# vmoens/mujoco-torch

Hardware: AMD Instinct MI355X
Metric: env-steps/sec (higher is better)
Workload: dtype f64

## Files before the change

mujoco-torch_amd/csrc/mjh_kernels.h:

```cpp
#pragma once
#include <cstring>
#include "mjh_device.h"

template <typename REAL>
struct LdsView {
  REAL* base;
  const LdsOff* off;
#define X(n, c, p) __device__ __forceinline__ REAL* n() const { return base + off->n; }
  MJH_LDS_ARRAYS(X, _)
#undef X
};

#ifndef MJH_NO_NT
#define MJH_NT_STORE(v, p) __builtin_nontemporal_store((v), (p))
#else
#define MJH_NT_STORE(v, p) (*(p) = (v))
#endif
template <typename MM>
inline int lds_carve(const MM& m, int phase_bit, LdsOff& o, int* kv_defer_ok = nullptr) {
  int off = 0;
#define X(n, c, p) o.n = off; if ((p) & phase_bit) off += (((c) + 1) & ~1);
  MJH_LDS_ARRAYS(X, m)
#undef X
  if (phase_bit == PH_CON) {
// ... 1543 lines not shown
          b[0] = 0; b[1] = 0; b[2] = 0;
          if ((REAL)-0.5 < n[1] && n[1] < (REAL)0.5) b[1] = 1; else b[2] = 1;
        }
        REAL c[3];
        cross3(n, b, c);
#pragma unroll
        for (int i = 0; i < 3; i++) { frame[i] = n[i]; frame[3 + i] = b[i]; frame[6 + i] = c[i]; }
        const REAL seg[3] = {axis[0] * s2[1], axis[1] * s2[1], axis[2] * s2[1]};
#pragma unroll
        for (int q = 0; q < 2; q++) {
          REAL sp[3];
#pragma unroll
          for (int i = 0; i < 3; i++) sp[i] = p2[i] + (q == 0 ? seg[i] : -seg[i]);
          plane_sphere_(n, p1, sp, s2[0], dist[q], pos[q]);
        }
      } else if (fn == MJH_FN_SPHERE_SPHERE) {
        REAL n[3];
        sphere_sphere_(p1, s1[0], p2, s2[0], dist[0], pos[0], n);
        make_frame(n, frame);
      } else if (fn == MJH_FN_SPHERE_CAPSULE) {
        const REAL axis[3] = {m2[2], m2[5], m2[8]};
        REAL a[3], b[3], pt[3], n[3];
#pragma unroll
        for (int i = 0; i < 3; i++) { REAL sg = axis[i] * s2[1]; a[i] = p2[i] - sg; b[i] = p2[i] + sg; }
        closest_segment_point(a, b, p1, pt);
        sphere_sphere_(p1, s1[0], pt, s2[0], dist[0], pos[0], n);
        make_frame(n, frame);
      } else if (fn == MJH_FN_CAPSULE_CAPSULE) {
        const REAL ax1[3] = {m1[2], m1[5], m1[8]}, ax2[3] = {m2[2], m2[5], m2[8]};
        REAL a0[3], a1[3], b0[3], b1[3], pt1[3], pt2[3], n[3];
#pragma unroll
        for (int i = 0; i < 3; i++) {
          REAL sg1 = ax1[i] * s1[1], sg2 = ax2[i] * s2[1];
          a0[i] = p1[i] - sg1; a1[i] = p1[i] + sg1; b0[i] = p2[i] - sg2; b1[i] = p2[i] + sg2;
        }
        closest_segment_to_segment(a0, a1, b0, b1, pt1, pt2);
        sphere_sphere_(pt1, s1[0], pt2, s2[0], dist[0], pos[0], n);
        make_frame(n, frame);
      } else {
        dist[0] = dist[1] = 1;
        for (int i = 0; i < 3; i++) pos[0][i] = pos[1][i] = 0;
        for (int i = 0; i < 9; i++) frame[i] = 0;
      }
      for (int q = 0; q < k && q < 2; q++) {
        const int c = M.pair_dst[p * MJH_MAX_PAIR_CONTACTS + q];
        S.con_dist()[c] = dist[q];
        for (int i = 0; i < 3; i++) S.con_pos()[3 * c + i] = pos[q][i];
        for (int i = 0; i < 9; i++) S.con_frame()[9 * c + i] = frame[i];
      }
    }
    wave_sync();
    STAMP(20);
    if (FRIC && M.topk) {
      const int nk = M.ncon, ncand = M.ncand;
      for (int q = l; q < ncand; q += W) {
        const REAL dq = S.con_dist()[q];
        int rank = 0;
        for (int q2 = 0; q2 < ncand; q2++) { const REAL d2 = S.con_dist()[q2]; rank += (d2 < dq) || (d2 == dq && q2 < q); }
        if (rank < nk) con_src_lds()[M.topk_slot[rank]] = q;
      }
      wave_sync();
      for (int c = l; c < nk; c += W) {
        const int q = con_src_lds()[c];
        if (out.contact_dist) out.contact_dist[e * nk + c] = S.con_dist()[q];
        for (int i = 0; i < 3; i++) if (out.contact_pos) out.contact_pos[(e * nk + c) * 3 + i] = S.con_pos()[3 * q + i];
        for (int i = 0; i < 9; i++) if (out.contact_frame) out.contact_frame[(e * nk + c) * 9 + i] = S.con_frame()[9 * q + i];
        if (out.contact_includemargin) out.contact_includemargin[e * nk + c] = M.con_includemargin[q];
        for (int i = 0; i < 5; i++) if (out.contact_friction) out.contact_friction[(e * nk + c) * 5 + i] = M.con_friction[5 * q + i];
        for (int i = 0; i < 2; i++) if (out.contact_solref) out.contact_solref[(e * nk + c) * 2 + i] = M.con_solref[2 * q + i];
        for (int i = 0; i < 2; i++) if (out.contact_solreffriction) out.contact_solreffriction[(e * nk + c) * 2 + i] = M.con_solreffriction[2 * q + i];
        for (int i = 0; i < 5; i++) if (out.contact_solimp) out.contact_solimp[(e * nk + c) * 5 + i] = M.con_solimp[5 * q + i];
        if (out.contact_dim) out.contact_dim[e * nk + c] = M.con_dim[q];
        if (out.contact_geom1) out.contact_geom1[e * nk + c] = M.con_geom1[q];
        if (out.contact_geom2) out.contact_geom2[e * nk + c] = M.con_geom2[q];
        if (out.contact_geom) { out.contact_geom[(e * nk + c) * 2] = M.con_geom1[q]; out.contact_geom[(e * nk + c) * 2 + 1] = M.con_geom2[q]; }
        if (out.contact_efc_address) out.contact_efc_address[e * nk + c] = M.con_efc_address[c];
      }
      return;
    }
    {
      const int nc = M.ncon;
      if (M.nt_all) putnt(out.contact_dist, S.con_dist(), nc); else put(out.contact_dist, S.con_dist(), nc);
      putnt(out.contact_pos, S.con_pos(), 3 * nc); putnt(out.contact_frame, S.con_frame(), 9 * nc);
      STAMP(21);
      if constexpr (PRE_NMAX > 0 || DEFER_CONST) return;
      contact_const_stores();
    }
  }
  __device__ __forceinline__ void contact_const_stores() {
    const int l = lane_here();
    if (!(out.contact_includemargin || out.contact_solref || out.contact_solreffriction || out.contact_friction || out.contact_solimp || out.contact_dim || out.contact_geom1 ||
          out.contact_geom2 || out.contact_geom || out.contact_efc_address)) return;
    {
      const int nc = M.ncon;
      {
        REAL* const dst[3] = {out.contact_includemargin, out.contact_solref, out.contact_solreffriction};
        const REAL* const src[3] = {M.con_includemargin, M.con_solref, M.con_solreffriction};
        const int cnt[3] = {nc, 2 * nc, 2 * nc};
        multi_copy_const<W, 3, 4>(dst, src, cnt, e);
      }
      {
        REAL* const dst[1] = {out.contact_friction};
        const REAL* const src[1] = {M.con_friction};
        const int cnt[1] = {5 * nc};
        multi_copy_const<W, 1, 10>(dst, src, cnt, e);
      }
      {
        REAL* const dst[1] = {out.contact_solimp};
        const REAL* const src[1] = {M.con_solimp};
        const int cnt[1] = {5 * nc};
        multi_copy_const<W, 1, 10>(dst, src, cnt, e);
      }
      for (int c0 = l; c0 < nc; c0 += 2 * W) {
        const int c1 = c0 + W;
        const bool h1 = c1 < nc;
        const int dim0 = M.con_dim[c0], g10 = M.con_geom1[c0], g20 = M.con_geom2[c0], adr0 = M.con_efc_address[c0];
        const int dim1 = h1 ? M.con_dim[c1] : 0, g11 = h1 ? M.con_geom1[c1] : 0, g21 = h1 ? M.con_geom2[c1] : 0, adr1 = h1 ? M.con_efc_address[c1] : 0;
        if (out.contact_dim) { out.contact_dim[e * nc + c0] = dim0; if (h1) out.contact_dim[e * nc + c1] = dim1; }
        if (out.contact_geom1) { out.contact_geom1[e * nc + c0] = g10; if (h1) out.contact_geom1[e * nc + c1] = g11; }
        if (out.contact_geom2) { out.contact_geom2[e * nc + c0] = g20; if (h1) out.contact_geom2[e * nc + c1] = g21; }
        if (out.contact_geom) {
          out.contact_geom[(e * nc + c0) * 2] = g10; out.contact_geom[(e * nc + c0) * 2 + 1] = g20;
          if (h1) { out.contact_geom[(e * nc + c1) * 2] = g11; out.contact_geom[(e * nc + c1) * 2 + 1] = g21; }
        }
        if (out.contact_efc_address) { out.contact_efc_address[e * nc + c0] = adr0; if (h1) out.contact_efc_address[e * nc + c1] = adr1; }
      }
    }
  }
  __device__ __forceinline__ int* con_src_lds() const { return reinterpret_cast<int*>(S.i_con_src()); }
  __device__ __forceinline__ int con_src(int c) const { return (FRIC && M.topk) ? con_src_lds()[c] : c; }

  template <bool BIG = false>
  __device__ __forceinline__ void jac_dof(const REAL* point, int body, int dof, REAL* jp, REAL* jr) const {
    const REAL on = BIG ? (REAL)((M.body_dofmask[body * M.mask_words + (dof >> 6)] >> (dof & 63)) & 1ull) : (REAL)((M.body_dofmask[body] >> dof) & 1ull);
    const REAL* rc = S.subtree_com() + 3 * M.body_rootid[body];
    const REAL off[3] = {point[0] - rc[0], point[1] - rc[1], point[2] - rc[2]};
    const REAL* cd = S.cdof() + 6 * dof;
    REAL c[3];
    cross3(cd, off, c);
#pragma unroll
    for (int i = 0; i < 3; i++) { jp[i] = (cd[3 + i] + c[i]) * on; jr[i] = cd[i] * on; }
  }

  __device__ __forceinline__ void jac_dof_root(const REAL* point, int root, REAL on, int dof, REAL* jp, REAL* jr) const {
    const REAL* rc = S.subtree_com() + 3 * root;
    const REAL off[3] = {point[0] - rc[0], point[1] - rc[1], point[2] - rc[2]};
    const REAL* cd = S.cdof() + 6 * dof;
    REAL c[3];
    cross3(cd, off, c);
#pragma unroll
    for (int i = 0; i < 3; i++) { jp[i] = (cd[3 + i] + c[i]) * on; jr[i] = cd[i] * on; }
  }

  __device__ __forceinline__ void kbi(const REAL* solref, const REAL* solimp, REAL pos, REAL& k, REAL& b, REAL& imp) const {
    REAL timeconst = solref[0], dampratio = solref[1];
    if (!(M.disableflags & DSBL_REFSAFE)) {
      const REAL t2 = 2 * M.timestep;
      timeconst = (timeconst > t2 ? timeconst : t2) * (REAL)(timeconst > 0);
    }
    REAL dmin = solimp[0], dmax = solimp[1], width = solimp[2], mid = solimp[3], power = solimp[4];
    auto clampf = [](REAL x, REAL lo, REAL hi) { return x < lo ? lo : (x > hi ? hi : x); };
    dmin = clampf(dmin, (REAL)mjMINIMP, (REAL)mjMAXIMP);
    dmax = clampf(dmax, (REAL)mjMINIMP, (REAL)mjMAXIMP);
    width = width > (REAL)MINVAL_CACHED ? width : (REAL)MINVAL_CACHED;
    mid = clampf(mid, (REAL)mjMINIMP, (REAL)mjMAXIMP);
    power = power > 1 ? power : (REAL)1;
    REAL kk = 1 / (dmax * dmax * timeconst * timeconst * dampratio * dampratio);
    REAL bb = 2 / (dmax * timeconst);
    if (dampratio <= 0) kk = -dampratio / (dmax * dmax);
    if (timeconst <= 0) bb = -timeconst / dmax;
    const REAL imp_x = r_abs(pos) / width;
    const bool sq = (power == (REAL)2);
    const REAL om = 1 - mid, ox = 1 - imp_x;
    const REAL pm = sq ? mid : r_pow<REAL>(mid, power - 1), pom = sq ? om : r_pow<REAL>(om, power - 1);
    const REAL px = sq ? imp_x * imp_x : r_pow<REAL>(imp_x, power), pox = sq ? ox * ox : r_pow<REAL>(ox, power);
    const REAL imp_a = (1 / pm) * px;
    const REAL imp_b = 1 - (1 / pom) * pox;
    const REAL imp_y = imp_x < mid ? imp_a : imp_b;
    REAL im = dmin + imp_y * (dmax - dmin);
    im = clampf(im, dmin, dmax);
    if (imp_x > 1) im = dmax;
    k = kk; b = bb; imp = im;
  }

  __device__ __forceinline__ void make_constraint() {
    const int l = lane_here();
    const int nv = M.nv, nefc = M.nefc, nl = M.nl, nf = FRIC ? M.nf : 0, nft = FRIC ? M.nft : 0, nfa = nf + nft, ne = FRIC ? M.ne : 0, nlb = FRIC ? M.nlb : 0, nlt = FRIC ? M.nlt : 0;
    if (nefc == 0) return;
    const int jrow0 = FRIC ? 0 : nl;
    const REAL* gq = KA.cur.qpos + e * M.nq;
    if (FRIC) { for (int i = l; i < M.nq; i += W) S.qpos_con()[i] = gq[i]; }
    {
      const bool from_in = !KA.state_from_cur;
      if (!con_inputs_loaded_) {
        REAL* const dst[3] = {S.qvel(), S.subtree_com(), S.cdof()};
        const REAL* const src[3] = {from_in ? in.qvel : KA.cur.qvel, out.subtree_com, out.cdof};
        const int cnt[3] = {nv, 3 * M.nbody, 6 * nv};
        multi_load<W, 3, 3>(dst, src, cnt, e);
      }
      if (from_in && KA.do_step) for (int i = l; i < nv; i += W) S.qvel()[i] = checked(S.qvel()[i], (REAL)0);
    }
    if (FRIC) for (int w = l; w < (ne + nfa + nlb + nl + nlt) * nv; w += W) S.efc_J()[w] = 0;
    wave_sync();
    STAMP(23);
    for (int w = l; w < (FRIC ? M.neqtab : 0) * nv; w += W) {
      int q, d;
      split_index(w, nv, M.inv_nv, q, d);
      const int kind = M.eq_kind[q], id = M.eq_id[q], id1 = M.eq_obj1[q], id2 = M.eq_obj2[q], row = M.eq_row[q];
      const REAL* data = M.eq_data + 11 * id;
      const REAL active = (REAL)in.eq_active[e * M.neq + id];
      if (kind == 2) {
        if (d != 0) continue;
        const int* ja = M.eq_jadr + 4 * q;
        const REAL has2 = (REAL)(id2 > -1);
        const REAL pos1 = S.qpos_con()[ja[2]], pos2 = S.qpos_con()[ja[3]] * has2;
        const REAL ref1 = M.qpos0[ja[2]], ref2 = M.qpos0[ja[3]] * has2;
        const REAL dif = pos2 - ref2;
        REAL pw[5];
#pragma unroll
        for (int i = 0; i < 5; i++) pw[i] = r_pow<REAL>(dif, (REAL)i);
        REAL deriv = 0, poly = 0;
#pragma unroll
        for (int i = 0; i < 4; i++) deriv += data[1 + i] * pw[i] * (REAL)(i + 1);
#pragma unroll
        for (int i = 0; i < 5; i++) poly += data[i] * pw[i];
        S.efc_J()[row * nv + ja[0]] = 1 * active;
        S.efc_J()[row * nv + ja[1]] = -deriv * active;
        const REAL pos = (pos1 - ref1 - poly) * active;
        S.efc_pos()[row] = pos;
        S.efc_pos_norm()[row] = pos;
        S.efc_invweight()[row] = M.dof_invweight0[ja[0]] + M.dof_invweight0[ja[1]] * has2;
        continue;
      }
      const int nb = M.nbody;
      const REAL *xm1 = out.xmat + (e * nb + id1) * 9, *xm2 = out.xmat + (e * nb + id2) * 9;
      const REAL *xp1 = out.xpos + (e * nb + id1) * 3, *xp2 = out.xpos + (e * nb + id2) * 3;
      const REAL* a1 = kind == 0 ? data : data + 3;
      const REAL* a2 = kind == 0 ? data + 3 : data;
      REAL pos1[3], pos2[3], cpos[3];
#pragma unroll
      for (int i = 0; i < 3; i++) {
        pos1[i] = ((xm1[3 * i] * a1[0] + xm1[3 * i + 1] * a1[1]) + xm1[3 * i + 2] * a1[2]) + xp1[i];
        pos2[i] = ((xm2[3 * i] * a2[0] + xm2[3 * i + 1] * a2[1]) + xm2[3 * i + 2] * a2[2]) + xp2[i];
        cpos[i] = pos1[i] - pos2[i];
      }
      REAL jp1[3], jr1[3], jp2[3], jr2[3];
      jac_dof<FRIC>(pos1, id1, d, jp1, jr1);
      jac_dof<FRIC>(pos2, id2, d, jp2, jr2);
#pragma unroll
      for (int i = 0; i < 3; i++) S.efc_J()[(row + i) * nv + d] = (jp1[i] - jp2[i]) * active;
      const REAL iwt = M.body_invweight0[id1] + M.body_invweight0[id2];
      if (kind == 0) {
        if (d == 0) {
          const REAL nrm = norm_n<REAL, 3>(cpos);
#pragma unroll
          for (int i = 0; i < 3; i++) { S.efc_pos()[row + i] = cpos[i] * active; S.efc_pos_norm()[row + i] = nrm * active; S.efc_invweight()[row + i] = iwt; }
        }
        continue;
      }
      const REAL torquescale = data[10];
      const REAL *xq1 = out.xquat + (e * nb + id1) * 4, *xq2 = out.xquat + (e * nb + id2) * 4;
      const REAL q1[4] = {xq1[0], xq1[1], xq1[2], xq1[3]}, rel[4] = {data[6], data[7], data[8], data[9]};
      REAL quat[4], qd[4];
      quat_mul(q1, rel, quat);
      const REAL quat1[4] = {xq2[0], xq2[1] * (REAL)-1, xq2[2] * (REAL)-1, xq2[3] * (REAL)-1};
      const REAL ax[3] = {(jr1[0] - jr2[0]) * torquescale, (jr1[1] - jr2[1]) * torquescale, (jr1[2] - jr2[2]) * torquescale};
      const REAL t[4] = {-quat1[1] * ax[0] - quat1[2] * ax[1] - quat1[3] * ax[2], quat1[0] * ax[0] + quat1[2] * ax[2] - quat1[3] * ax[1],
                         quat1[0] * ax[1] + quat1[3] * ax[0] - quat1[1] * ax[2], quat1[0] * ax[2] + quat1[1] * ax[1] - quat1[2] * ax[0]};
      REAL o[4];
      quat_mul(t, quat, o);
#pragma unroll
      for (int i = 0; i < 3; i++) S.efc_J()[(row + 3 + i) * nv + d] = ((REAL)0.5 * o[1 + i]) * active;
      if (d == 0) {
        quat_mul(quat1, quat, qd);
        const REAL pos6[6] = {cpos[0], cpos[1], cpos[2], qd[1] * torquescale, qd[2] * torquescale, qd[3] * torquescale};
        const REAL nrm = norm_n<REAL, 6>(pos6);
        const REAL iwr = M.body_invweight0_rot[id1] + M.body_invweight0_rot[id2];
#pragma unroll
        for (int i = 0; i < 6; i++) { S.efc_pos()[row + i] = pos6[i] * active; S.efc_pos_norm()[row + i] = nrm * active; S.efc_invweight()[row + i] = i < 3 ? iwt : iwr; }
      }
    }
    for (int r0 = l; r0 < nf; r0 += W) {
      const int r = ne + r0;
      const int da = M.fric_dof[r0];
      S.efc_J()[r * nv + da] = 1;
      S.efc_pos()[r] = 0;
      S.efc_pos_norm()[r] = 0;
      S.efc_invweight()[r] = M.dof_invweight0[da];
    }
    for (int r0 = l; r0 < nft; r0 += W) {
      const int r = ne + nf + r0;
      const int t = M.fric_tendon[r0];
      for (int d = 0; d < nv; d++) S.efc_J()[r * nv + d] = M.ten_J0[t * nv + d];
      S.efc_pos()[r] = 0;
      S.efc_pos_norm()[r] = 0;
      S.efc_invweight()[r] = M.tendon_invweight0[t];
    }
    for (int r0 = l; r0 < nlb; r0 += W) {
      const int r = ne + nfa + r0;
      const int j = M.lim_ball_jnt[r0], qa = M.jnt_qposadr[j], da = M.jnt_dofadr[j];
      const REAL q[4] = {S.qpos_con()[qa], S.qpos_con()[qa + 1], S.qpos_con()[qa + 2], S.qpos_con()[qa + 3]};
      REAL axis[3], angle;
      quat_to_axis_angle(q, axis, angle);
      const REAL r0_ = M.jnt_range[2 * j], r1_ = M.jnt_range[2 * j + 1];
      const REAL pos = ((r0_ > r1_ ? r0_ : r1_) - angle) - M.jnt_margin[j];
      const REAL active = (REAL)(pos < 0);
// ... 1496 lines not shown
          const REAL gradient = r_sqrt<REAL>(gg) / scale;
          bool done = c.niter >= M.iterations;
          done |= improvement < (REAL)M.tolerance;
          done |= gradient < (REAL)M.tolerance;
          if (done) break;
        }
        do_init = false; do_ls = true; do_grad = !(it + 1 >= M.iterations);
      }
      if (do_ls) {
        linesearch(c);
        STAMP(60);
        for (int d = l; d < nv; d += W) { S.s_pgrad()[d] = S.s_grad()[d]; S.s_pMgrad()[d] = S.s_Mgrad()[d]; }
        wave_sync();
      }
      if (do_init) {
        for (int d = l; d < nv; d += W) S.s_qacc()[d] = src[d];
        wave_sync();
        mul_J(S.s_qacc(), S.s_Jaref(), S.efc_aref());
        if (ph == P_SMOOTH) {
          for (int d = l; d < nv; d += W) S.s_Ma()[d] = 0;
        } else {
          mul_M(S.s_qacc(), S.s_Ma());
        }
        c.gauss = 0; c.cost = (REAL)INFINITY; c.prev_cost = 0; c.niter = 0;
        for (int d = l; d < nv; d += W) { S.s_grad()[d] = 0; S.s_Mgrad()[d] = 0; S.s_search()[d] = 0; }
        wave_sync();
      }
      STAMP(68);
      if (do_ls || do_init) update_constraint(c);
      STAMP(67);
      if (ph >= P_START) constraint_qfrc();
      STAMP(66);
      if (do_grad) {
        update_gradient();
        if (ph == P_START || M.solver == SOL_NEWTON) {
          for (int d = l; d < nv; d += W) S.s_search()[d] = -S.s_Mgrad()[d];
        } else {
          REAL num = 0, den = 0;
          for (int d = l; d < nv; d += W) { num += S.s_grad()[d] * (S.s_Mgrad()[d] - S.s_pMgrad()[d]); den += S.s_pgrad()[d] * S.s_pMgrad()[d]; }
          num = wave_sum(num); den = wave_sum(den);
          REAL beta = num / (den > (REAL)mjMINVAL ? den : (REAL)mjMINVAL);
          beta = beta > 0 ? beta : (REAL)0;
          for (int d = l; d < nv; d += W) S.s_search()[d] = -S.s_Mgrad()[d] + beta * S.s_search()[d];
        }
        wave_sync();
      }
      if (ph == P_SMOOTH) { smooth_cost = c.cost; ph = P_WARM; }
      else if (ph == P_WARM) { use_warm = __builtin_amdgcn_readfirstlane((int)(c.cost < smooth_cost)) != 0; ph = P_START; STAMP(54); }
      else if (ph == P_START) { ph = P_ITER; STAMP(55); }
      else { c.niter++; it++; }
    }
    for (int d = l; d < nv; d += W) { S.qacc()[d] = S.s_qacc()[d]; S.qacc_warm()[d] = S.s_qacc()[d]; S.qfrc_constraint()[d] = S.s_qfrc()[d]; }
    wave_sync();
    STAMP(61);
    put(out.qacc, S.qacc(), nv); put(out.qacc_warmstart, S.qacc(), nv); put(out.qfrc_constraint, S.qfrc_constraint(), nv);
    if (out.efc_force) {
      const int c0 = nf_() + M.nl + nft_() + ne_() + nlim_rows();
      for (int r = l; r < c0; r += W) out.efc_force[e * nefc + ext_row(r)] = S.s_force()[r];
      for (int r = l; r < nefc - c0; r += W) { const int q = row_dst_lds()[r]; out.efc_force[e * nefc + c0 + r] = q >= 0 ? S.s_force()[c0 + q] : (REAL)0; }
    }
    STAMP(62);
  }

  __device__ __forceinline__ void integrate_pos(const REAL* qpos, const REAL* qvel, REAL dt, REAL* o) {
    for (int j = lane(); j < M.njnt; j += W) {
      const int t = M.jnt_type[j], qa = M.jnt_qposadr[j], da = M.jnt_dofadr[j];
      if (t == JNT_FREE) {
        for (int i = 0; i < 3; i++) o[qa + i] = qpos[qa + i] + dt * qvel[da + i];
        REAL q[4] = {qpos[qa + 3], qpos[qa + 4], qpos[qa + 5], qpos[qa + 6]}, w[3] = {qvel[da + 3], qvel[da + 4], qvel[da + 5]}, r[4];
        quat_integrate(q, w, dt, r);
        for (int i = 0; i < 4; i++) o[qa + 3 + i] = r[i];
      } else if (t == JNT_BALL) {
        REAL q[4] = {qpos[qa], qpos[qa + 1], qpos[qa + 2], qpos[qa + 3]}, w[3] = {qvel[da], qvel[da + 1], qvel[da + 2]}, r[4];
        quat_integrate(q, w, dt, r);
        for (int i = 0; i < 4; i++) o[qa + i] = r[i];
      } else {
        o[qa] = qpos[qa] + dt * qvel[da];
      }
    }
  }

  __device__ __forceinline__ void advance_act(const REAL* act0, const REAL* act_dot, REAL* dst) {
    const REAL dt = M.timestep;
    for (int i = lane(); i < M.nu; i += W) {
      const int dyn = M.act_dyntype[i];
      if (dyn == DYN_NONE) continue;
      const int a = M.act_actadr[i];
      REAL act = act0[a];
      if (dyn == DYN_FILTEREXACT) {
        REAL tau = M.act_dynprm[3 * i];
        tau = tau > (REAL)mjMINVAL ? tau : (REAL)mjMINVAL;
        act = act + act_dot[a] * tau * (1 - r_exp<REAL>(-dt / tau));
      } else {
        act = act + act_dot[a] * dt;
      }
      if (M.act_actlimited[i]) {
        const REAL lo = M.act_actrange[2 * i], hi = M.act_actrange[2 * i + 1];
        act = act < lo ? lo : (act > hi ? hi : act);
      }
      if (dst) dst[e * M.na + a] = act;
    }
  }

  __device__ __forceinline__ void advance(const REAL* qpos0, const REAL* qvel0, const REAL* act0, REAL time0, const REAL* act_dot, const REAL* qacc, const REAL* qvel_for_pos) {
    const int l = lane_here();
    const REAL dt = M.timestep;
    const StatePtrs<REAL>& fin = KA.fin;
    advance_act(act0, act_dot, fin.act);
    for (int d = l; d < M.nv; d += W) S.tmp_nv()[d] = qvel0[d] + qacc[d] * dt;
    wave_sync();
    integrate_pos(qpos0, qvel_for_pos ? qvel_for_pos : S.tmp_nv(), dt, S.tmp_nq());
    wave_sync();
    row_store<W>(fin.qpos, S.tmp_nq(), M.nq, e);
    row_store<W>(fin.qvel, S.tmp_nv(), M.nv, e);
    if (l == 0 && fin.time) fin.time[e] = time0 + dt;
  }

  template <bool DEFER = false, bool KEEPG = false, bool XK = KEEPG>
  __device__ __forceinline__ void run_kin() {
    STAMP0();
    load_qpos(true);
    wave_sync();
    STAMP(1);
    const bool com_first = XK && (__builtin_popcount((unsigned)blockIdx.x & (unsigned)KA.xswap_k) & 1) != 0;
    kinematics<DEFER, KEEPG, XK>(KA.rk_stage <= 0, com_first);
    if (!com_first) com_pos<DEFER, KEEPG>();
  }
  __device__ __forceinline__ void run_crb() { crb_factor<false>(); }
  __device__ __forceinline__ void run_con() {
    STAMP0();
    if (M.ncon > 0) collision<0, false, true>();
    if (KA.stages & 0x78) make_constraint();
    if (M.ncon > 0 && !(FRIC && M.topk) && !consts_done_) contact_const_stores();
  }
  template <int NMAX>
  __device__ __forceinline__ void sol2_prefetch(Sol2Pre<REAL, NMAX>& P) {
    const int l = lane_here();
    const int nq = M.nq, nv = M.nv, na = M.na;
    const bool dof = l < nv;
    P.f = (dof && out.qfrc_smooth) ? out.qfrc_smooth[e * nv + l] : (REAL)0;
    {
      const REAL* gL = out.qLD + e * nv * nv;
#pragma unroll
      for (int k = 0; k < NMAX; k++) P.T.t[k] = (dof && k < nv) ? (k <= l ? gL[l * nv + k] : gL[k * nv + l]) : (REAL)0;
    }
    P.T.inv = 0;
    const REAL* gq = KA.cur.qpos + e * nq;
#pragma unroll
    for (int j = 0; j < 2; j++) P.qp[j] = l + W * j < nq ? gq[l + W * j] : (REAL)0;
    P.ac = 0; P.ad = 0;
    if (l < na) { const REAL* ga = KA.state_from_cur ? KA.cur.act : in.act; P.ac = ga ? ga[e * na + l] : (REAL)0; P.ad = out.act_dot ? out.act_dot[e * na + l] : (REAL)0; }
    P.warm = (dof && KA.warm_src && M.nefc > 0) ? KA.warm_src[e * nv + l] : (REAL)0;
  }
  template <int NMAX>
  __device__ __forceinline__ void make_constraint_cs(Sol2Pre<REAL, NMAX>& pre, Sol2Con<REAL>& C) {
    const int l = lane_here();
#if MJH_CS_PF >= 2
    {
      const REAL* gq = KA.cur.qpos + e * M.nq;
#pragma unroll
      for (int j = 0; j < 2; j++) pre.qp[j] = l + W * j < M.nq ? gq[l + W * j] : (REAL)0;
    }
#endif
    const int nv = M.nv, nefc = M.nefc, nl = M.nl, ncon = M.ncon, rows = M.con_rows;
    const bool elliptic = M.cone == CONE_ELLIPTIC;
    if (!KA.state_from_cur && KA.do_step) for (int i = l; i < nv; i += W) S.qvel()[i] = checked(S.qvel()[i], (REAL)0);
    REAL lpos = 0, linvw = 0;
    int lj = 0;
    C.jl = 0; C.ldof = 0;
    if (l < nl) {
      lj = M.lim_jnt[l];
      C.ldof = M.jnt_dofadr[lj];
    }
    {
      const int qa = l < nl ? M.jnt_qposadr[lj] : 0;
      const int srcl = (int)(lane_id() & ~(W - 1)) + (qa & (W - 1));
      const REAL q0 = __shfl(pre.qp[0], srcl, MJH_WAVE), q1 = __shfl(pre.qp[1], srcl, MJH_WAVE);
      const REAL q = qa < W ? q0 : q1;
      if (l < nl) {
        const REAL dist_min = q - M.jnt_range[2 * lj], dist_max = M.jnt_range[2 * lj + 1] - q;
        const REAL val = (REAL)(dist_min < dist_max) * 2 - 1;
        const REAL pos = (dist_min < dist_max ? dist_min : dist_max) - M.jnt_margin[lj];
        const REAL active = (REAL)(pos < 0);
        C.jl = val * active;
        lpos = pos * active;
        linvw = M.dof_invweight0[C.ldof];
      }
    }
    int* const act_list = reinterpret_cast<int*>(S.i_con_act());
    int* const slot = reinterpret_cast<int*>(S.i_crow_act());
    int nact = 0;
    for (int base = 0; base < ncon; base += W) {
      const int c = base + l;
      const bool valid = c < ncon;
      const bool act = valid && (S.con_dist()[valid ? c : 0] - M.con_includemargin[valid ? c : 0]) < 0;
      int tot;
      const int at = sub_prefix_count<W>(act, tot) + nact;
      if (act) act_list[at] = c;
      if (valid) slot[c] = act ? at : -1;
      nact += tot;
    }
    C.nact = nact;
    C.nda = nact * rows;
    wave_sync();
    STAMP(23);
    REAL* const Jc = S.efc_Jc();
    for (int w = l; w < nact * nv; w += W) {
      int a, d;
      split_index(w, nv, M.inv_nv, a, d);
      const int c = act_list[a];
      const int dim = M.con_dim[c];
      const int* cb = M.con_body + 4 * c;
      const int root1 = cb[2], root2 = cb[3];
      const REAL on1 = (REAL)((M.con_dmask[2 * c] >> d) & 1ull), on2 = (REAL)((M.con_dmask[2 * c + 1] >> d) & 1ull);
      const REAL* fr = S.con_frame() + 9 * c;
      const REAL* cpos = S.con_pos() + 3 * c;
      const REAL* fric = M.con_friction + 5 * c;
      REAL jp1[3], jr1[3], jp2[3], jr2[3];
      jac_dof_root(cpos, root2, on2, d, jp2, jr2);
      jac_dof_root(cpos, root1, on1, d, jp1, jr1);
      const REAL dp[3] = {jp2[0] - jp1[0], jp2[1] - jp1[1], jp2[2] - jp1[2]};
      const REAL dr[3] = {jr2[0] - jr1[0], jr2[1] - jr1[1], jr2[2] - jr1[2]};
      REAL diff[6];
#pragma unroll
      for (int r = 0; r < 3; r++) {
        diff[r] = fr[3 * r] * dp[0] + fr[3 * r + 1] * dp[1] + fr[3 * r + 2] * dp[2];
        diff[3 + r] = fr[3 * r] * dr[0] + fr[3 * r + 1] * dr[1] + fr[3 * r + 2] * dr[2];
      }
      REAL* const dst = Jc + (a * rows) * nv + d;
      if (dim == 1) {
        dst[0] = diff[0];
      } else if (!elliptic) {
        const int nedge = 2 * (dim - 1);
        for (int ed = 0; ed < nedge; ed++) {
          const REAL f = fric[ed >> 1] * ((ed & 1) ? (REAL)-1 : (REAL)1);
          dst[ed * nv] = diff[0] + diff[1 + (ed >> 1)] * f;
        }
      } else {
        for (int r = 0; r < dim; r++) dst[r * nv] = diff[r];
      }
    }
#if MJH_CS_PF == 2
    sol2_prefetch<NMAX>(pre);
#endif
    wave_sync();
    STAMP(25);
    C.Dl = 0; C.arl = 0;
    for (int r = l; r < nefc; r += W) {
      REAL solref[2], solimp[5];
      REAL pos = 0, pos_norm = 0, invweight = 0, jv = 0;
      int crow = -1;
      if (r < nl) {
        pos = lpos; pos_norm = lpos; invweight = linvw;
        solref[0] = M.jnt_solref[2 * lj]; solref[1] = M.jnt_solref[2 * lj + 1];
#pragma unroll
        for (int i = 0; i < 5; i++) solimp[i] = M.jnt_solimp[5 * lj + i];
        jv = 0 + C.jl * S.qvel()[C.ldof];
      } else {
        const int q = r - nl, ncr = M.ncrow;
        const int info = M.crow_info[q];
        const REAL* P = M.crow_par + q;
        solref[0] = P[0]; solref[1] = P[ncr];
#pragma unroll
        for (int i = 0; i < 5; i++) solimp[i] = P[(2 + i) * ncr];
        invweight = P[7 * ncr];
        const int c = info & 0xffff, sub = (info >> 16) & 0xff;
        const REAL dist = S.con_dist()[c] - P[8 * ncr];
        const REAL active = (REAL)(dist < 0);
        if (!(info >> 24)) { pos = dist * active; pos_norm = dist * active; }
        else { pos = (sub == 0 ? dist : (REAL)0) * active; pos_norm = dist; }
        if (dist < 0) {
          crow = slot[c] * rows + sub;
          jv = dot_seq(Jc + crow * nv, 1, S.qvel(), 1, nv);
        }
      }
      REAL k, b, imp;
      kbi(solref, solimp, pos_norm, k, b, imp);
      REAL rr = invweight * (1 - imp) / imp;
      rr = rr > (REAL)MINVAL_CACHED ? rr : (REAL)MINVAL_CACHED;
      const REAL aref_r = -b * jv - k * imp * pos, D_r = 1 / rr;
      if (out.efc_aref) MJH_NT_STORE(aref_r, &out.efc_aref[e * nefc + r]);
      if (out.efc_D) MJH_NT_STORE(D_r, &out.efc_D[e * nefc + r]);
      if (r < nl) { C.Dl = D_r; C.arl = aref_r; }
      else if (crow >= 0) { S.efc_aref()[crow] = aref_r; S.efc_D()[crow] = D_r; }
    }
    STAMP(26);
  }
  __device__ __forceinline__ void cs_deferred_stores(const Sol2Con<REAL>& C) {
    const int l = lane_here();
    const int nv = M.nv, nefc = M.nefc, nl = M.nl, nd = nefc - nl, rows = M.con_rows;
    rebind();
    if (out.efc_J) {
      REAL* gJ = out.efc_J + e * nefc * nv;
      const bool dof = l < nv;
      for (int r = 0; r < nl; r++) {
        const int col = sub_read<W>(C.ldof, r);
        const REAL v = sub_read<W>(C.jl, r);
        if (dof) MJH_NT_STORE((l == col) ? v : (REAL)0, &gJ[r * nv + l]);
      }
      const int* slot = reinterpret_cast<const int*>(S.i_crow_act());
      const REAL* Jc = S.efc_Jc();
      REAL* gC = gJ + nl * nv;
      for (int c = 0; c < M.ncon; c++) {
        const int at = slot[c];
        for (int sub = 0; sub < rows; sub += 4) {
          REAL v[4];
#pragma unroll
          for (int t = 0; t < 4; t++) v[t] = (at >= 0 && sub + t < rows && dof) ? Jc[(at * rows + sub + t) * nv + l] : (REAL)0;
#pragma unroll
          for (int t = 0; t < 4; t++) if (sub + t < rows && dof) MJH_NT_STORE(v[t], &gC[(c * rows + sub + t) * nv + l]);
        }
      }
    }
    if (out.efc_frictionloss) for (int r = l; r < nefc; r += W) MJH_NT_STORE((REAL)0, &out.efc_frictionloss[e * nefc + r]);
    if (M.ncon > 0) contact_const_stores();
  }
  template <int NMAX, int RPL, bool ONE = false, bool HANDOFF = false>
  __device__ __forceinline__ void run_con_sol2() {
    static_assert(W == 32 && !FRIC && !DIRECT, "plain constraint stage, two environments per wavefront");
    Sol2Pre<REAL, NMAX> pre;
    Sol2Con<REAL> con;
    STAMP0();
    collision<NMAX, HANDOFF>(&pre);
#if MJH_CS_PF == 1
    sol2_prefetch<NMAX>(pre);
#endif
    make_constraint_cs<NMAX>(pre, con);
#if MJH_CS_PF == 3
    if (HANDOFF && ho_on_) {
      __builtin_amdgcn_fence(__ATOMIC_RELEASE, "workgroup");
      __builtin_amdgcn_fence(__ATOMIC_ACQUIRE, "workgroup");
    }
    sol2_prefetch<NMAX>(pre);
#endif
    wave_sync();
    run_sol2<NMAX, RPL, false, true, ONE>(&pre, &con);
  }
  template <bool FLUID, bool FUSED = false, bool DEFER = false, bool BATCH = false>
  __device__ __forceinline__ void run_vel() {
    STAMP0();
    velocity<FLUID, FUSED, DEFER, BATCH>();
    if (KA.stages & 0x60) actuation<FLUID>();
    velocity_stores<DEFER>();
  }

  __device__ __forceinline__ void run_sol() {
    const int l = lane_here();
    const int nq = M.nq, nv = M.nv, na = M.na;
    STAMP0();
    load_factor_and_accelerate((KA.stages & 0x40) != 0);
    if (!(KA.stages & 0x40)) return;
    STAMP(53);
    if (M.nefc == 0) {
      for (int d = l; d < nv; d += W) S.qacc()[d] = S.qacc_smooth()[d];
      wave_sync();
      put(out.qacc, S.qacc(), nv);
    } else {
      solve();
    }
    integrate_tail();
  }

  template <int NMAX>
  __device__ __forceinline__ void load_damping_rows(TriPack<REAL, NMAX>& Hh) {
    const int l = lane_here();
    const int nv = M.nv;
    const REAL* gM = out.qM + e * nv * nv;
#pragma unroll
    for (int k = 0; k < NMAX; k++) Hh.t[k] = (l < nv && k <= l) ? gM[k * nv + l] : (REAL)0;
  }
  template <int NLO = 0, int NHI = (1 << 30)>
  __device__ __forceinline__ void integrate_tail() {
    const int l = lane_here();
    const int nq = M.nq, nv = M.nv, na = M.na;
    if (!KA.do_step) return;
    rebind();
    const REAL dt = M.timestep;
    const REAL time0 = in.time ? in.time[e] : (REAL)0;
    const int rk = KA.rk_stage;
    if (rk < 0) {
      const REAL* qacc = S.qacc();
      constexpr bool REGSOL = NHI <= 32;
      if (!(M.disableflags & DSBL_EULERDAMP)) {
        if constexpr (REGSOL && NLO > 16) {
          TriPack<REAL, NHI> Hh;
          load_damping_rows<NHI>(Hh);
          const REAL dd = l < nv ? M.timestep * M.dof_damping[l] : (REAL)0;
          const REAL rhs = l < nv ? S.qfrc_smooth()[l] + (M.nefc ? S.qfrc_constraint()[l] : (in.qfrc_constraint ? in.qfrc_constraint[e * nv + l] : (REAL)0)) : (REAL)0;
#pragma unroll
          for (int k = 0; k < NHI; k++) Hh.t[k] = (k == l) ? Hh.t[k] + dd : Hh.t[k];
          chol_pack_big<W, REAL, NHI>(Hh, S.chol_col(), nv);
          const REAL x = tri_solve<W, REAL, NHI>(Hh, rhs, nv);
          if (l < nv) S.s_Mgrad()[l] = x;
          wave_sync();
        } else {
        REAL* const Hp = REGSOL ? S.H2() : S.H();
        for (int w = l; w < (nv * (nv + 1)) / 2; w += W) {
          int i, j;
          tri_unpack(w, i, j);
          const REAL mw = out.qM[e * nv * nv + i * nv + j];
          Hp[w] = (i == j) ? mw + M.timestep * M.dof_damping[i] : mw;
        }
        for (int d = l; d < nv; d += W) S.s_grad()[d] = S.qfrc_smooth()[d] + (M.nefc ? S.qfrc_constraint()[d] : (in.qfrc_constraint ? in.qfrc_constraint[e * nv + d] : (REAL)0));
        wave_sync();
        if (NLO <= 16 && (NHI <= 16 || nv <= 16)) {
          if constexpr (NLO <= 16) chol_factor_solve<W, REAL, NLO, (NHI < 16 ? NHI : 16)>(Hp, S.s_grad(), S.s_Mgrad(), nv);
        } else {
          if constexpr (NHI > 16 && !REGSOL) {
            chol_factor<W, REAL, 16, true>(S.H(), S.HL(), nv);
            chol_inv_diag<W, false>(S.HL(), S.HL_inv(), nv);
            wave_sync();
            chol_solve<W, false>(S.HL(), S.HL_inv(), S.s_grad(), S.s_Mgrad(), nv);
          }
        }
        }
        qacc = S.s_Mgrad();
      }
      advance(S.qpos(), S.qvel(), S.act(), time0, S.act_dot(), qacc, nullptr);
      return;
    }
    const REAL A[3] = {(REAL)0.5, (REAL)0.5, (REAL)1.0};
    const REAL Bt[4] = {(REAL)(float)(1.0 / 6.0), (REAL)(float)(1.0 / 3.0), (REAL)(float)(1.0 / 3.0), (REAL)(float)(1.0 / 6.0)};
    const RkWork<REAL>& RW = KA.W;
    const REAL b = Bt[rk];
    for (int i = l; i < nv; i += W) {
      const REAL kq = S.qvel()[i], qa = S.qacc()[i];
      if (rk == 0) { RW.qvel0[e * nv + i] = kq; RW.sum_qvel[e * nv + i] = b * kq; RW.sum_qacc[e * nv + i] = b * qa; }
      else { RW.sum_qvel[e * nv + i] = RW.sum_qvel[e * nv + i] + b * kq; RW.sum_qacc[e * nv + i] = RW.sum_qacc[e * nv + i] + b * qa; }
    }
    for (int i = l; i < na; i += W) {
      const REAL ad = S.act_dot()[i];
      if (rk == 0) { RW.act0[e * na + i] = S.act()[i]; RW.sum_actdot[e * na + i] = b * ad; }
      else RW.sum_actdot[e * na + i] = RW.sum_actdot[e * na + i] + b * ad;
    }
    const REAL* qpos0g = KA.fin.qpos + e * nq;
    for (int i = l; i < nq; i += W) S.tmp_nq()[i] = (rk == 0) ? S.qpos()[i] : qpos0g[i];
    for (int i = l; i < nv; i += W) S.s_pgrad()[i] = (rk == 0) ? S.qvel()[i] : RW.qvel0[e * nv + i];
    for (int i = l; i < na; i += W) S.act()[i] = (rk == 0) ? S.act()[i] : RW.act0[e * na + i];
    wave_sync();
    if (rk < 3) {
      const REAL a = A[rk];
      for (int i = l; i < nv; i += W) S.tmp_nv2()[i] = a * S.qvel()[i];
      wave_sync();
      for (int i = l; i < nq; i += W) S.qpos()[i] = S.tmp_nq()[i];
      wave_sync();
      integrate_pos(S.qpos(), S.tmp_nv2(), dt, S.tmp_nq());
      for (int i = l; i < na; i += W) KA.nxt.act[e * na + i] = S.act()[i] + (a * S.act_dot()[i]) * dt;
      for (int i = l; i < nv; i += W) KA.nxt.qvel[e * nv + i] = S.s_pgrad()[i] + (a * S.qacc()[i]) * dt;
      wave_sync();
      row_store<W>(KA.nxt.qpos, S.tmp_nq(), nq, e);
      return;
    }
    for (int i = l; i < nv; i += W) { S.s_mv()[i] = RW.sum_qacc[e * nv + i]; S.tmp_nv2()[i] = RW.sum_qvel[e * nv + i]; }
    for (int i = l; i < na; i += W) S.act_dot()[i] = RW.sum_actdot[e * na + i];
    for (int i = l; i < nq; i += W) S.qpos()[i] = S.tmp_nq()[i];
    wave_sync();
    advance(S.qpos(), S.s_pgrad(), S.act(), time0, S.act_dot(), S.s_mv(), S.tmp_nv2());
  }

  template <int NMAX>
  __device__ __forceinline__ REAL tri_solve2(const TriPack<REAL, NMAX>& T, REAL bi) const {
    return tri_solve<W, REAL, NMAX>(T, bi, M.nv);
  }

  template <int NMAX, int RPL, bool NEWTON_ONLY = false, bool CS = false, bool ONE = false>
  __device__ __forceinline__ void run_sol2(const Sol2Pre<REAL, NMAX>* pre = nullptr, const Sol2Con<REAL>* con = nullptr) {
    static_assert(W == 32 || W == 16, "two or four environments per wavefront");
    static_assert(!CS || (W == 32 && !NEWTON_ONLY), "the fused constraint + solver kernel runs two environments per wavefront");
    constexpr bool NEWT = NMAX <= 16;
    const int l = lane_here();
    const int nq = M.nq, nv = M.nv, na = M.na, nefc = M.nefc, nl = M.nl, nd = nefc - nl;
    const bool dof = l < nv, lim = l < nl;
    const bool solving = (KA.stages & 0x40) != 0;
    const bool from_in = !KA.state_from_cur;
    const bool newton = NEWTON_ONLY ? NEWT : (NEWT && M.solver == SOL_NEWTON);
    STAMP0();
    if (KA.row_lo >= 0 && !KA.scan_marks) {
      int rows_active = 0;
      if (solving && nefc > 0) {
        const int ncon = M.ncon;
// ... 969 lines not shown
```

Before: 31.09 million.

## Compute contact Jacobian per DOF lane with chunked software-prefetched contact data

Adds a BYDOF path for building the active-contact Jacobian. Each lane owns one DOF and holds its cdof row in registers, then loops over active contacts in chunks of four, loading the next contact's position, frame and root COMs while computing the current one. This replaces the flattened contact×DOF index loop with its per-element index split and repeated cdof loads. The new path is enabled only when HANDOFF is set. It serialises work over contacts per lane, so lanes with l >= nv sit idle, and the extra per-contact staging raises register pressure.

```diff
diff --git a/mujoco-torch_amd/csrc/mjh_kernels.h b/mujoco-torch_amd/csrc/mjh_kernels.h
--- a/mujoco-torch_amd/csrc/mjh_kernels.h
+++ b/mujoco-torch_amd/csrc/mjh_kernels.h
@@ -1719,6 +1719,14 @@
     for (int i = 0; i < 3; i++) { jp[i] = (cd[3 + i] + c[i]) * on; jr[i] = cd[i] * on; }
   }
 
+  __device__ __forceinline__ static void jac_dof_vals(const REAL* point, const REAL* rc, const REAL* cd, REAL on, REAL* jp, REAL* jr) {
+    const REAL off[3] = {point[0] - rc[0], point[1] - rc[1], point[2] - rc[2]};
+    REAL c[3];
+    cross3(cd, off, c);
+#pragma unroll
+    for (int i = 0; i < 3; i++) { jp[i] = (cd[3 + i] + c[i]) * on; jr[i] = cd[i] * on; }
+  }
+
   __device__ __forceinline__ void kbi(const REAL* solref, const REAL* solimp, REAL pos, REAL& k, REAL& b, REAL& imp) const {
     REAL timeconst = solref[0], dampratio = solref[1];
     if (!(M.disableflags & DSBL_REFSAFE)) {
@@ -3521,7 +3529,7 @@
     if (l < na) { const REAL* ga = KA.state_from_cur ? KA.cur.act : in.act; P.ac = ga ? ga[e * na + l] : (REAL)0; P.ad = out.act_dot ? out.act_dot[e * na + l] : (REAL)0; }
     P.warm = (dof && KA.warm_src && M.nefc > 0) ? KA.warm_src[e * nv + l] : (REAL)0;
   }
-  template <int NMAX>
+  template <int NMAX, bool BYDOF = false>
   __device__ __forceinline__ void make_constraint_cs(Sol2Pre<REAL, NMAX>& pre, Sol2Con<REAL>& C) {
     const int l = lane_here();
 #if MJH_CS_PF >= 2
@@ -3574,6 +3582,86 @@
     wave_sync();
     STAMP(23);
     REAL* const Jc = S.efc_Jc();
+    if constexpr (BYDOF) {
+      const bool dof = l < nv;
+      const int d = dof ? l : 0;
+      REAL cd[6];
+#pragma unroll
+      for (int i = 0; i < 6; i++) cd[i] = S.cdof()[6 * d + i];
+      const int* const tab_dim = M.con_dim;
+      const int* const tab_body = M.con_body;
+      const unsigned long long* const tab_mask = M.con_dmask;
+      const REAL* const tab_fric = M.con_friction;
+      const REAL* const sc = S.subtree_com();
+      const REAL* const cfr = S.con_frame();
+      const REAL* const cps = S.con_pos();
+      constexpr int CH = 4;
+      constexpr int NF = 2;
+      for (int a0 = 0; a0 < nact; a0 += CH) {
+        int cc[CH], dims[CH], rt1[CH], rt2[CH], bit1[CH], bit2[CH];
+        REAL fr_k[CH][NF];
+#pragma unroll
+        for (int t = 0; t < CH; t++) cc[t] = act_list[a0 + t < nact ? a0 + t : a0];
+#pragma unroll
+        for (int t = 0; t < CH; t++) {
+          const int c = cc[t];
+          dims[t] = tab_dim[c];
+          rt1[t] = tab_body[4 * c + 2]; rt2[t] = tab_body[4 * c + 3];
+          bit1[t] = (int)((tab_mask[2 * c] >> d) & 1ull); bit2[t] = (int)((tab_mask[2 * c + 1] >> d) & 1ull);
+#pragma unroll
+          for (int k = 0; k < NF; k++) fr_k[t][k] = tab_fric[5 * c + k];
+        }
+        REAL nx[18];
+        auto request = [&](int t) {
+#pragma unroll
+          for (int i = 0; i < 3; i++) nx[i] = cps[3 * cc[t] + i];
+#pragma unroll
+          for (int i = 0; i < 9; i++) nx[3 + i] = cfr[9 * cc[t] + i];
+#pragma unroll
+          for (int i = 0; i < 3; i++) { nx[12 + i] = sc[3 * rt2[t] + i]; nx[15 + i] = sc[3 * rt1[t] + i]; }
+        };
+        request(0);
+#pragma unroll
+        for (int t = 0; t < CH; t++) {
+          if (a0 + t >= nact) break;
+          REAL cu[18];
+#pragma unroll
+          for (int i = 0; i < 18; i++) cu[i] = nx[i];
+          if (t + 1 < CH) request(t + 1);
+          const REAL* const cpos = cu;
+          const REAL* const fr = cu + 3;
+          const int dim = dims[t];
+          REAL jp1[3], jr1[3], jp2[3], jr2[3];
+          jac_dof_vals(cpos, cu + 12, cd, (REAL)bit2[t], jp2, jr2);
+          jac_dof_vals(cpos, cu + 15, cd, (REAL)bit1[t], jp1, jr1);
+          const REAL dp[3] = {jp2[0] - jp1[0], jp2[1] - jp1[1], jp2[2] - jp1[2]};
+          const REAL dr[3] = {jr2[0] - jr1[0], jr2[1] - jr1[1], jr2[2] - jr1[2]};
+          REAL diff[6];
+#pragma unroll
+          for (int r = 0; r < 3; r++) {
+            diff[r] = fr[3 * r] * dp[0] + fr[3 * r + 1] * dp[1] + fr[3 * r + 2] * dp[2];
+            diff[3 + r] = fr[3 * r] * dr[0] + fr[3 * r + 1] * dr[1] + fr[3 * r + 2] * dr[2];
+          }
+          if (dof) {
+            REAL* const dst = Jc + ((a0 + t) * rows) * nv + d;
+            if (dim == 1) {
+              dst[0] = diff[0];
+            } else if (!elliptic) {
+#pragma unroll
+              for (int k = 0; k < 5; k++) {
+                if (k >= dim - 1) break;
+                const REAL fk = k < NF ? fr_k[t][k < NF ? k : 0] : tab_fric[5 * cc[t] + k];
+                dst[(2 * k) * nv] = diff[0] + diff[1 + k] * (fk * (REAL)1);
+                dst[(2 * k + 1) * nv] = diff[0] + diff[1 + k] * (fk * (REAL)-1);
+              }
+            } else {
+#pragma unroll
+              for (int r = 0; r < 6; r++) if (r < dim) dst[r * nv] = diff[r];
+            }
+          }
+        }
+      }
+    } else
     for (int w = l; w < nact * nv; w += W) {
       int a, d;
       split_index(w, nv, M.inv_nv, a, d);
@@ -3694,7 +3782,7 @@
 #if MJH_CS_PF == 1
     sol2_prefetch<NMAX>(pre);
 #endif
-    make_constraint_cs<NMAX>(pre, con);
+    make_constraint_cs<NMAX, HANDOFF>(pre, con);
 #if MJH_CS_PF == 3
     if (HANDOFF && ho_on_) {
       __builtin_amdgcn_fence(__ATOMIC_RELEASE, "workgroup");
```

After: 31.82 million, median of 6. 1.02x the previous value.
